# Patryk27/strolle

Hardware: NVIDIA H100
Metric: Mrays/s (+ frames/s) at 1080p-per-GPU Cornell, ReSTIR DI+GI + SVGF; H100 vs CPU restatement of the reference (higher is better)
Workload: dtype f32

## Files before the change

strolle_b200/csrc/engine.cu:

```cuda
#include <algorithm>
#include <cmath>
#include <cstdio>
#include <cstring>
#include <deque>
#include <functional>
#include <limits>
#include <string>
#include <unordered_map>
#include <vector>

#include <nccl.h>

#include "../../include/strolle_b200.h"
#include "kernels.h"

#include <dlfcn.h>
namespace {
struct NcclApi {
    void* lib = nullptr;
    ncclResult_t (*GetUniqueId)(ncclUniqueId*) = nullptr;
    ncclResult_t (*CommInitRank)(ncclComm_t*, int, ncclUniqueId, int) = nullptr;
    ncclResult_t (*CommDestroy)(ncclComm_t) = nullptr;
    ncclResult_t (*GroupStart)() = nullptr;
    ncclResult_t (*GroupEnd)() = nullptr;
// ... 305 lines not shown
    void* p = nullptr; size_t cap = 0;
    int ensure(size_t bytes) {
        if (bytes <= cap) return ST_OK;
        if (p) cudaFree(p);
        p = nullptr; cap = 0;
        size_t want = std::max<size_t>(bytes, 256);
        CK(cudaMalloc(&p, want));
        CK(cudaMemset(p, 0, want));
        CK(cudaDeviceSynchronize());
        cap = want;
        return ST_OK;
    }
    void release() { if (p) cudaFree(p); p = nullptr; cap = 0; }
};

static const char* kPassNames[P_COUNT] = {
    "prim_gbuffer", "di_sampling", "di_temporal_resampling", "di_spatial_resampling_pick", "di_spatial_resampling_trace", "di_spatial_resampling_sample",
    "di_resolving", "gi_reprojection", "gi_sampling_a", "gi_sampling_b", "gi_temporal_resampling", "gi_spatial_resampling_pick",
    "gi_spatial_resampling_trace", "gi_spatial_resampling_sample", "gi_preview_resampling", "gi_resolving", "frame_reprojection",
    "frame_denoising_reproject", "frame_denoising_estimate_variance", "frame_denoising_wavelet", "frame_composition", "ref_tracing",
    "ref_shading", "bvh_heatmap", "atmosphere", "trace_stream", "halo_exchange"};

static uint32_t dispatch_seed(uint32_t base, uint32_t frame, uint32_t k) {
    uint32_t s = base ^ (frame * 64u + k);
    s = s * 747796405u + 2891336453u;
    uint32_t w = ((s >> ((s >> 28) + 4u)) ^ s) * 277803737u;
    return (w >> 22) ^ w;
}

static const ExposureDev kExposureDefaults = {0.0f, 0.0f, -8.0f, 8.0f, 0.1f, 0.9f, 0.05f, 1.0f / 60.0f};
static const BloomDev kBloomDefaults = {0.15f, 0.7f, 0.0f, 0.0f, 7, 0};
static const st_depth_of_field kDofDefaults = {10.0f, 1.0f, 0.01866f, 16.0f};

struct CameraSlot {
    bool alive = false;
    st_camera desc;
    st_camera prev_desc;
    uint32_t frame = 0;
    CameraDev dev;
    std::vector<std::pair<std::string, float4**>> named;
    std::vector<std::pair<std::string, size_t>> sizes;
    DevMem arena;
    DevMem svgf_pairs; float4* pair[2] = {nullptr, nullptr};
    DevMem rgba8; int rgba8_slot = 0;
    DevMem taa; float4* taa_hist[2] = {nullptr, nullptr};
    DevMem expo;
    DevMem bloom;
    DevMem dof;
    cudaEvent_t ev_ready[2] = {nullptr, nullptr}, ev_copied[2] = {nullptr, nullptr};
    cudaStream_t side[2] = {nullptr, nullptr}; cudaEvent_t ev_produced = nullptr, ev_pushed[2] = {nullptr, nullptr}; bool pushed_pending[2] = {false, false};
    struct PeerLink { bool ready = false; bool ipc = false; std::vector<char*> arena, rgba8; std::vector<uint32_t*> flags; DevMem sync; uint32_t seq = 0, fseq = 0; } peer;
};

struct Step { int pass; std::function<void(cudaStream_t)> run; int sub = -1; };

}

using namespace st;

struct st_engine {
    int device = 0;
    cudaStream_t stream = nullptr; bool own_stream = true;
    cudaStream_t copy_stream = nullptr;
    std::unordered_map<st_handle, std::vector<st_mesh_triangle>> meshes;
    std::vector<st_material> materials; std::vector<st_handle> material_handles; bool materials_dirty = false;
    struct MatTex { st_handle tex[4]; uint32_t mask; };
    std::vector<MatTex> material_textures;
    struct ImageRect { st_handle handle; uint32_t x, y, w, h; };
    std::vector<ImageRect> images; uint32_t shelf_x = 0, shelf_y = 0, shelf_h = 0; bool images_dirty = false;
    DevMem d_atlas, d_srgb, d_tri_instance, d_instance_xforms;
    bool motion_dirty = true;
    bool moved_last_tick = false;
    struct Inst {
        st_handle handle, mesh, material; Affine3 xf, xf_inv, prev_xf; bool dirty;
        st_handle baked_mesh = ~(st_handle)0, baked_material = ~(st_handle)0; bool host_stale = false; Affine3 dev_xf, dev_xf_inv;
    };
    std::vector<Inst> instances; bool instances_dirty = false;
    struct Range { st_handle handle; size_t b, e; };
    std::vector<Range> tri_ranges; SlotAllocator tri_alloc;
    std::vector<float4> h_triangles; std::vector<Prim> prims; bool triangles_dirty = false;
    BvhBuild bvh; BvhOut bvh_out; bool bvh_dirty = false;
    std::vector<GpuMaterial> h_materials;
    static const st_handle kSun = ~(st_handle)0;
    std::vector<GpuLight> h_lights; std::vector<std::pair<st_handle, uint32_t>> light_slots;
    std::vector<st_handle> lights_created, lights_updated; std::vector<std::pair<st_handle, uint32_t>> lights_remapped; std::vector<uint32_t> lights_killed;
    uint32_t next_light = 1; bool lights_dirty = true;
    float sun_azimuth = 0.0f, sun_altitude = 0.35f; bool sun_dirty = true;
    GpuWorld world;
    uint32_t frame = 1, seed_base = 0xC0FFEEu;
    DevMem d_triangles, d_bvh, d_materials, d_matpacked, d_unpacklut, d_lights, d_noise, d_tlut, d_slut, d_skylut, d_scratch, d_raycount;
    bool count_rays = false;
    bool svgf_fast = true;
    bool shading_fast = ST_SHADING_FAST_DEFAULT != 0;
    bool fused_passes = ST_FUSED_PASSES_DEFAULT != 0;
    bool async_output = false;
    bool halo_nccl = false;
    int wavelet_paired = ST_WAVELET_PAIRED_DEFAULT;
    int strip_dma = ST_STRIP_DMA_DEFAULT;
    bool strip_fused = true;
    bool last_frame_fused = false;
    int wavelet_tiled = ST_WAVELET_TILED_DEFAULT;
    int wavelet_cfg = ST_WAVELET_CFG_DEFAULT;
    DevMem d_tile_errors; uint64_t wavelet_tiled_launches = 0;
    bool fuse_reproject = ST_FUSE_REPROJECT_DEFAULT != 0;
    bool bvh_reuse = true;
    bool variance_tiled = ST_VARIANCE_TILED_DEFAULT != 0; uint64_t variance_tiled_launches = 0;
    bool normal_maps = false, any_normal_map = false, nmap_frame = false; uint64_t normal_map_launches = 0;
    int bvh_refit = 0; uint32_t refit_run = 0; uint64_t bvh_refits = 0; bool structure_changed = false;
    RefitPlan plan; bool plan_ready = false; std::vector<uint32_t> plan_levels; std::vector<uint8_t> plan_alpha; DevMem d_plan, d_bake;
    std::unordered_map<st_handle, DevMem> d_meshes;
    void* staging[2] = {nullptr, nullptr}; size_t staging_cap[2] = {0, 0}; cudaEvent_t staging_ev[2] = {nullptr, nullptr}; int staging_slot = 0;
    int light_grid = 0, lgrid_built = 0; bool lgrid_frame = false; LightGridDev lgrid{}; DevMem d_lgrid; uint64_t light_grid_builds = 0;
    bool texture_filter = false, texf_built = false, any_color_texture = false, texf_frame = false; TexFilterDev texf{};
    DevMem d_texf_pool, d_texf_table, d_texf_jobs; std::vector<uint2> h_texf_table; std::vector<MipJob> h_texf_jobs; size_t texf_pool_texels = 0;
    uint64_t texture_mip_builds = 0;
    bool temporal_aa = false, taa_frame = false; uint64_t taa_resolves = 0;
// ... 521 lines not shown
    const double fx = -(double)c.transform[8], fy = -(double)c.transform[9], fz = -(double)c.transform[10];
    const double n = std::sqrt(fx * fx + fy * fy + fz * fz);
    DofDev p = {};
    p.active = active ? 1 : 0; p.k = (float)k; p.F = l.focal_distance; p.R = l.max_radius;
    p.fwd_x = (float)(fx / n); p.fwd_y = (float)(fy / n); p.fwd_z = (float)(fz / n);
    p.reach = (int)std::ceil((double)l.max_radius / kDofTile);
    const DofBufs b = dof_bufs(cs);
    const float fl[8] = {(float)f, (float)A, p.k, p.F, p.R, p.fwd_x, p.fwd_y, p.fwd_z};
    p.head[0] = c.width; p.head[1] = c.height; p.head[2] = (uint32_t)b.tx; p.head[3] = (uint32_t)b.ty; p.head[4] = (uint32_t)p.active;
    std::memcpy(p.head + 5, fl, sizeof fl);
    return p;
}
static bool lens_params(const st_engine* e, const CameraSlot* cs, uint32_t seed, LensDev* out) {
    const st_depth_of_field& l = e->dof_cfg;
    const st_camera& c = cs->desc;
    const double f = 0.5 * (double)l.sensor_height * (double)c.projection[5], A = f / (double)l.aperture_f_stops;
    if (!(e->dof_frame && c.mode == ST_MODE_REFERENCE && (double)l.focal_distance > f)) return false;
    double ax[3][3];
    for (int k = 0; k < 3; k++) {
        const double sg = k == 2 ? -1.0 : 1.0;
        const double x = sg * c.transform[4 * k], y = sg * c.transform[4 * k + 1], z = sg * c.transform[4 * k + 2], n = std::sqrt(x * x + y * y + z * z);
        ax[k][0] = x / n; ax[k][1] = y / n; ax[k][2] = z / n;
    }
    *out = LensDev{seed, (float)(A / 2.0), l.focal_distance, (float)ax[0][0], (float)ax[0][1], (float)ax[0][2], (float)ax[1][0], (float)ax[1][1],
                   (float)ax[1][2], (float)ax[2][0], (float)ax[2][1], (float)ax[2][2]};
    return true;
}
static CameraDev frame_source(const st_engine* e, const CameraSlot* cs, CameraDev c) {
    if (defocuses(e, cs) && cs->dof.p) c.output = dof_bufs(cs).frame;
    return c;
}
static void build_schedule(st_engine* e, CameraSlot* cs, std::vector<Step>* steps, const StripExt* ext = nullptr) {
    GpuCamera jc, jp; float4 jit;
    const bool taa = taa_cameras(e, cs, &jc, &jp, &jit);
    const CameraDev cam = [&] { CameraDev c = cs->dev; if (taa) { c.curr = jc; c.prev = jp; } return c; }();
    const StripExt no_ext; const StripExt& x = ext ? *ext : no_ext;
    const CameraDev camG = grown(cam, x.gbuffer), camV = grown(cam, x.variance);
    const int pm0 = x.preview_mirror[0], pm1 = x.preview_mirror[1];
    const SceneDev sc = e->scene();
    const uint32_t f = cs->frame;
    const int cur = (f % 2u) == 1u ? 1 : 0;
    const st_camera& d = cs->desc;
    const bool fs = e->shading_fast;
    const bool nm = e->nmap_frame;
    const bool lgon = e->lgrid_frame;
    const LightGridDev lgd = e->lgrid;
    const bool tfon = e->texf_frame;
    const TexFilterDev tfd = e->texf;
    const bool emon = e->envm_frame;
    EnvMapDev emd = e->envm;
    if (!e->envs_frame) emd.cdf = nullptr;
    const bool eson = emon && e->envs_frame;
    auto seed = [&](uint32_t k) { return dispatch_seed(e->seed_base, f, k); };
    auto add = [&](int pass, std::function<void(cudaStream_t)> fn) { steps->push_back(Step{pass, std::move(fn)}); };
    const CameraDev camO = frame_source(e, cs, cam);
    auto defocus = [&]() {
        if (!defocuses(e, cs)) return;
        const DofDev dp = dof_params(e, cs); const DofBufs db = dof_bufs(cs);
        add(P_COMPOSITION, [=](cudaStream_t s) { e->dof_gathers++; launch_depth_of_field(cam, dp, db, s); });
    };
    auto meter = [&]() {
        if (!meters(e, cs)) return;
        uint32_t* state = (uint32_t*)cs->expo.p; const ExposureDev ep = e->expo_frame; const int sms = e->sm_count;
        add(P_COMPOSITION, [=](cudaStream_t s) { e->exposure_meterings++; launch_exposure_histogram(camO, state, ep, sms, s); });
    };
    auto pyramid = [&]() {
        if (!blooms(e, cs)) return;
        const BloomLevels lv = bloom_levels(e, cs); const uint32_t* state = meters(e, cs) ? (const uint32_t*)cs->expo.p : nullptr;
        const ExposureDev ep = e->expo_frame; const int tm = e->tm_frame; const BloomDev bp = e->bloom_cfg;
        add(P_COMPOSITION, [=](cudaStream_t s) { e->bloom_pyramids++; launch_bloom_pyramid(camO, lv, state, ep, tm, bp, s); });
    };
    const float4* di_final = (d.denoise && (d.mode == ST_MODE_IMAGE || d.mode == ST_MODE_DI_DIFFUSE)) ? cam.di_diff_curr_colors : cam.di_diff_samples;
    const float4* gi_final = (d.denoise && (d.mode == ST_MODE_IMAGE || d.mode == ST_MODE_GI_DIFFUSE)) ? cam.gi_diff_curr_colors : cam.gi_diff_samples;
    if (d.mode == ST_MODE_BVH_HEATMAP) {
        add(P_BVH_HEATMAP, [=](cudaStream_t s) { launch_bvh_heatmap(cam, sc, s); });
        add(P_COMPOSITION, [=](cudaStream_t s) { launch_composition(cam, sc, cur, 5u, di_final, gi_final, s); });
        return;
    }
    if (d.mode == ST_MODE_REFERENCE) {
        LensDev lens;
        const bool lon = lens_params(e, cs, seed(K_LENS), &lens);
        for (uint32_t depth = 0; depth <= (uint32_t)d.ref_depth; depth++) {
            uint32_t sd = seed(P_REF_SHADING_SEED + depth);
            add(P_REF_TRACING, [=](cudaStream_t s) { if (nm) e->normal_map_launches++; launch_ref_tracing(cam, sc, depth, nm, lon ? &lens : nullptr, s); });
            add(P_REF_SHADING, [=](cudaStream_t s) {
                if (emon) e->envm_launches++;
                launch_ref_shading(cam, sc, sd, depth, lgon ? &lgd : nullptr, tfon ? &tfd : nullptr, emon ? &emd : nullptr, lon ? &lens : nullptr, s);
            });
        }
        add(P_REF_SHADING, [=](cudaStream_t s) { launch_ref_shading(cam, sc, 0u, 255u, nullptr, nullptr, nullptr, nullptr, s); });
        add(P_COMPOSITION, [=](cudaStream_t s) { launch_composition(cam, sc, cur, 6u, di_final, gi_final, s); });
        meter(); pyramid();
        return;
    }
    const bool needs_di = d.mode == ST_MODE_IMAGE || d.mode == ST_MODE_DI_DIFFUSE || d.mode == ST_MODE_DI_SPECULAR;
    const bool needs_gi = d.mode == ST_MODE_IMAGE || d.mode == ST_MODE_GI_DIFFUSE || d.mode == ST_MODE_GI_SPECULAR;
    const int k4_in_k0 = (e->fused_passes && (ext == nullptr || ext->still) && !e->instances.empty()) ? 1 : 0;
    add(P_PRIM_GBUFFER, [=](cudaStream_t s) { if (nm) e->normal_map_launches++; launch_prim_gbuffer(camG, sc, cur, k4_in_k0, nm, tfon ? &tfd : nullptr, s); });
    const bool fp = e->fused_passes;
    if (!e->instances.empty()) {
        if (!k4_in_k0) add(P_FRAME_REPROJECTION, [=](cudaStream_t s) { launch_frame_reprojection(cam, sc, cur, s); });
        if (needs_di) {
            uint32_t s1 = seed(P_DI_SAMPLING), s2 = seed(P_DI_TEMPORAL), s3 = seed(P_DI_SPATIAL_PICK), s5 = seed(P_DI_SPATIAL_SAMPLE);
            if (fp) {
                add(P_DI_TEMPORAL, [=](cudaStream_t s) { (fs ? stf::launch_di_sample_temporal : st::launch_di_sample_temporal)(cam, sc, cur, s1, s2, f, lgon ? &lgd : nullptr, s); });
                add(P_DI_SPATIAL_PICK, [=](cudaStream_t s) { (fs ? stf::launch_di_spatial_fused : st::launch_di_spatial_fused)(cam, sc, cur, s3, s5, f, s); });
            } else {
                add(P_DI_SAMPLING, [=](cudaStream_t s) { (fs ? stf::launch_di_sampling : st::launch_di_sampling)(cam, sc, cur, s1, f, lgon ? &lgd : nullptr, s); });
                add(P_DI_TEMPORAL, [=](cudaStream_t s) { (fs ? stf::launch_di_temporal : st::launch_di_temporal)(cam, sc, cur, s2, s); });
                add(P_DI_SPATIAL_PICK, [=](cudaStream_t s) { (fs ? stf::launch_di_spatial_pick : st::launch_di_spatial_pick)(cam, sc, cur, s3, f, s); });
                add(P_DI_SPATIAL_TRACE, [=](cudaStream_t s) { (fs ? stf::launch_spatial_trace : st::launch_spatial_trace)(cam, sc, cam.di_diff_samples, cam.di_diff_curr_colors, cam.di_diff_stash, s); });
                add(P_DI_SPATIAL_SAMPLE, [=](cudaStream_t s) { (fs ? stf::launch_di_spatial_sample : st::launch_di_spatial_sample)(cam, sc, s5, f, s); });
            }
            add(P_DI_RESOLVING, [=](cudaStream_t s) { if (emon) e->envm_launches++; (fs ? stf::launch_di_resolving : st::launch_di_resolving)(cam, sc, cur, emon ? &emd : nullptr, s); });
        }
        if (needs_gi) {
            uint32_t sa = seed(P_GI_SAMPLING_A), sb = seed(P_GI_SAMPLING_B), st_ = seed(P_GI_TEMPORAL), sp = seed(P_GI_SPATIAL_PICK), ss = seed(P_GI_SPATIAL_SAMPLE), sv = seed(P_GI_PREVIEW);
            uint32_t source;
            const bool tracing = f % 6u < 4u;
            const int inline_rp = (fp && tracing) ? 1 : 0;
            if (!inline_rp) add(P_GI_REPROJECTION, [=](cudaStream_t s) { (fs ? stf::launch_gi_reprojection : st::launch_gi_reprojection)(cam, sc, cur, s); });
            auto sampling = [&]() {
                if (fp) {
                    add(P_GI_SAMPLING_B, [=](cudaStream_t s) {
                        if (nm) e->normal_map_launches++;
                        if (emon) e->envm_launches++;
                        (fs ? stf::launch_gi_sampling_fused : st::launch_gi_sampling_fused)(cam, sc, cur, sa, sb, f, nm, lgon ? &lgd : nullptr, tfon ? &tfd : nullptr, emon ? &emd : nullptr, s);
                    });
                    return;
                }
                add(P_GI_SAMPLING_A, [=](cudaStream_t s) {
                    if (nm) e->normal_map_launches++;
                    if (eson) e->envm_launches++;
                    (fs ? stf::launch_gi_sampling_a : st::launch_gi_sampling_a)(cam, sc, cur, sa, f, nm, tfon ? &tfd : nullptr, eson ? &emd : nullptr, s);
                });
                add(P_GI_SAMPLING_B, [=](cudaStream_t s) { if (emon) e->envm_launches++; (fs ? stf::launch_gi_sampling_b : st::launch_gi_sampling_b)(cam, sc, cur, sb, f, lgon ? &lgd : nullptr, emon ? &emd : nullptr, s); });
            };
            if (tracing) {
                if (f % 2u == 0u) sampling();
                add(P_GI_TEMPORAL, [=](cudaStream_t s) { (fs ? stf::launch_gi_temporal : st::launch_gi_temporal)(cam, sc, cur, st_, f, inline_rp, s); });
                if (f % 2u == 1u) {
                    if (fp) add(P_GI_SPATIAL_PICK, [=](cudaStream_t s) { (fs ? stf::launch_gi_spatial_fused : st::launch_gi_spatial_fused)(cam, sc, cur, sp, ss, f, s); });
                    else {
                        add(P_GI_SPATIAL_PICK, [=](cudaStream_t s) { (fs ? stf::launch_gi_spatial_pick : st::launch_gi_spatial_pick)(cam, sc, cur, sp, f, s); });
                        add(P_GI_SPATIAL_TRACE, [=](cudaStream_t s) { (fs ? stf::launch_spatial_trace : st::launch_spatial_trace)(cam, sc, cam.gi_d0, cam.gi_d1, cam.gi_d2, s); });
                        add(P_GI_SPATIAL_SAMPLE, [=](cudaStream_t s) { (fs ? stf::launch_gi_spatial_sample : st::launch_gi_spatial_sample)(cam, sc, ss, f, s); });
                    }
                    source = 1;
                } else source = 0;
            } else {
                sampling();
                add(P_GI_TEMPORAL, [=](cudaStream_t s) { (fs ? stf::launch_gi_temporal : st::launch_gi_temporal)(cam, sc, cur, st_, f, 0, s); });
                source = 0;
            }
            const float4* src0 = source == 0 ? cam.gi_reservoirs[1] : cam.gi_reservoirs[2];
            add(P_GI_PREVIEW, [=](cudaStream_t s) { (fs ? stf::launch_gi_preview : st::launch_gi_preview)(cam, sc, cur, sv, 0u, src0, cam.gi_reservoirs[3], pm0, s); });
            if (fp) add(P_GI_PREVIEW, [=](cudaStream_t s) { (fs ? stf::launch_gi_preview_resolve : st::launch_gi_preview_resolve)(cam, sc, cur, sv, cam.gi_reservoirs[3], src0, s); });
            else {
                add(P_GI_PREVIEW, [=](cudaStream_t s) { (fs ? stf::launch_gi_preview : st::launch_gi_preview)(cam, sc, cur, sv, 1u, cam.gi_reservoirs[3], cam.gi_reservoirs[0], pm1, s); });
                add(P_GI_RESOLVING, [=](cudaStream_t s) { (fs ? stf::launch_gi_resolving : st::launch_gi_resolving)(cam, sc, cur, src0, s); });
            }
        }
    }
    if (d.denoise) {
        if (e->fuse_reproject) {
            add(P_DENOISE_REPROJECT, [=](cudaStream_t s) { launch_denoise_reproject_pair(cam, sc, cur, s); });
        } else {
            add(P_DENOISE_REPROJECT, [=](cudaStream_t s) { launch_denoise_reproject(cam, sc, cur, cam.di_diff_prev_colors, cam.di_diff_moments[cur ^ 1], cam.di_diff_samples, cam.di_diff_curr_colors, cam.di_diff_moments[cur], s); });
            add(P_DENOISE_REPROJECT, [=](cudaStream_t s) { launch_denoise_reproject(cam, sc, cur, cam.gi_diff_prev_colors, cam.gi_diff_moments[cur ^ 1], cam.gi_diff_samples, cam.gi_diff_curr_colors, cam.gi_diff_moments[cur], s); });
        }
        const bool fast = e->svgf_fast;
        const bool var_tiled = e->variance_tiled; uint32_t* verr = (uint32_t*)e->d_tile_errors.p;
        add(P_DENOISE_VARIANCE, [=](cudaStream_t s) {
            if (var_tiled && launch_denoise_variance_tiled(camV, sc, cur, fast, verr, s)) { e->variance_tiled_launches++; return; }
            launch_denoise_variance(camV, sc, cur, fast, s);
        });
        float4* di_io[5][2] = {{cam.di_diff_stash, cam.di_diff_prev_colors}, {cam.di_diff_prev_colors, cam.di_diff_stash}, {cam.di_diff_stash, cam.di_diff_curr_colors},
                               {cam.di_diff_curr_colors, cam.di_diff_stash}, {cam.di_diff_stash, cam.di_diff_curr_colors}};
        float4* gi_io[5][2] = {{cam.gi_diff_stash, cam.gi_diff_prev_colors}, {cam.gi_diff_prev_colors, cam.gi_diff_stash}, {cam.gi_diff_stash, cam.gi_diff_curr_colors},
                               {cam.gi_diff_curr_colors, cam.gi_diff_stash}, {cam.gi_diff_stash, cam.gi_diff_curr_colors}};
        const bool whole_or_fused = ext != nullptr || (cam.y0 == 0 && cam.y1 == cam.h);
        const int first_paired_read = (fast && whole_or_fused && cs->pair[0]) ? (e->wavelet_paired == 2 ? 3 : e->wavelet_paired == 1 ? 4 : 5) : 5;
        for (uint32_t nth = 0; nth < 5; nth++) {
            float4 *a = di_io[nth][0], *b = di_io[nth][1], *c = gi_io[nth][0], *g = gi_io[nth][1];
            const bool reads_pair = (int)nth >= first_paired_read, writes_pair = (int)nth + 1 >= first_paired_read && nth < 4;
            const float4* pin = reads_pair ? cs->pair[nth & 1] : nullptr; float4* pout = writes_pair ? cs->pair[(nth + 1) & 1] : nullptr;
            const bool tiled = !reads_pair && ((e->wavelet_tiled >> nth) & 1) != 0; const int cfg = (e->wavelet_cfg >> (4 * nth)) & 15;
            uint32_t* terr = (uint32_t*)e->d_tile_errors.p;
            const CameraDev camW = grown(cam, x.wavelet[nth]);
            add(P_DENOISE_WAVELET, [=](cudaStream_t s) {
                if (tiled && launch_denoise_wavelet_tiled(camW, sc, f, 1u << nth, (float)(1 + nth), a, b, c, g, pout, fast, cfg, terr, s)) { e->wavelet_tiled_launches++; return; }
                launch_denoise_wavelet(camW, sc, cur, f, 1u << nth, (float)(1 + nth), a, b, c, g, pin, pout, fast, s);
            });
            steps->back().sub = (int)nth;
        }
    }
    uint32_t mode = (uint32_t)d.mode;
    if (taa) {
        const float4* hin = cs->taa_hist[cur ^ 1]; float4* hout = cs->taa_hist[cur];
        add(P_COMPOSITION, [=](cudaStream_t s) { e->taa_resolves++; launch_taa_resolve(cam, sc, cur, mode, di_final, gi_final, hin, hout, jit, s); });
        defocus(); meter(); pyramid();
        return;
    }
    add(P_COMPOSITION, [=](cudaStream_t s) { launch_composition(cam, sc, cur, mode, di_final, gi_final, s); });
    defocus(); meter(); pyramid();
}


struct HaloItem { std::string name; int reach; };
struct HaloExchange { int before_step; std::vector<HaloItem> items; };
static const int kSpatialReach = 128;
static const int kPreview2Reach = 64;
static const int kVarianceReach = 3;
static const int kWaveletReach[5] = {1, 2, 4, 9, 19};

// ... 259 lines not shown
            break;
        case StripOp::PULL: {
            StripPull pl; std::memset(&pl, 0, sizeof pl);
            for (int r = 0; r < N; r++) { pl.arena[r] = cs->peer.arena[r]; pl.bounds[r] = bounds[r].first; }
            pl.bounds[N] = H; pl.n_ranks = N; pl.rank = R; pl.w = (int)cs->desc.width; pl.h = H; pl.own_y0 = d.own_y0; pl.own_y1 = d.own_y1;
            pl.need_rows = (const int*)(sync + kNeedRowsWord); pl.pulled_rows = (unsigned long long*)(sync + kPulledRowsWord);
            struct { std::string name; int local; } items[] = {
                {std::string("prim_surface_map_") + prv, kSpatialReach}, {std::string("prim_gbuffer_d0_") + prv, kSpatialReach}, {std::string("prim_gbuffer_d1_") + prv, kSpatialReach},
                {"di_reservoirs_0", 0}, {"gi_reservoirs_0", 0}, {"di_diff_prev_colors", 0}, {"gi_diff_prev_colors", 0},
                {std::string("di_diff_moments_") + prv, 0}, {std::string("gi_diff_moments_") + prv, 0}};
            for (auto& it : items) {
                size_t kk = 0; float4* base = camera_buffer(cs, it.name, &kk);
                if (!base) return fail(ST_ERR_NOT_FOUND, "pull list names unknown buffer " + it.name);
                pl.items[pl.nitems++] = StripPullItem{(size_t)((char*)base - (char*)cs->arena.p), (int)kk, it.local};
            }
            e->run_timed(P_HALO_EXCHANGE, [=](cudaStream_t s) { launch_strip_pull(pl, s); });
            break;
        }
        }
    }
    d.y0 = d.own_y0; d.y1 = d.own_y1;
    if (push_rc) return push_rc;
    CK(cudaGetLastError());
    return ST_OK;
}

static CameraSlot* get_camera(st_engine* e, st_camera_handle h) { return (h >= 0 && (size_t)h < e->cameras.size() && e->cameras[h]->alive) ? e->cameras[h] : nullptr; }

}

extern "C" {

int st_copy_output(st_engine* e, st_camera_handle h, void* host_out, int format);
const char* st_last_error(void) { return g_err.c_str(); }
const char* st_pass_name(int pass) { return (pass >= 0 && pass < P_COUNT) ? kPassNames[pass] : ""; }

int st_engine_create(int device, st_engine** out) {
    if (!out) return fail(ST_ERR_INVALID, "out is null");
    int count = 0;
    cudaError_t ce = cudaGetDeviceCount(&count);
    if (ce != cudaSuccess || count == 0) return fail(ST_ERR_CUDA, "no CUDA device available: this library has no CPU fallback");
    if (device < 0 || device >= count) return fail(ST_ERR_INVALID, "bad device ordinal");
    CK(cudaSetDevice(device));
    st_engine* e = new st_engine();
    e->device = device;
    CK(cudaDeviceGetAttribute(&e->sm_count, cudaDevAttrMultiProcessorCount, device));
    CK(cudaStreamCreateWithFlags(&e->stream, cudaStreamNonBlocking));
    std::memset(&e->world, 0, sizeof e->world);
    e->h_lights.push_back(make_sun(make_float4(0, 0, 0, 25.0f), make_float4(0, 0, 0, std::numeric_limits<float>::infinity())));
    e->light_slots.push_back({st_engine::kSun, 0u});
    int rc = e->d_noise.ensure(256 * 256 * 4); if (rc) { delete e; return rc; }
    rc = e->d_unpacklut.ensure(512 * 4); if (rc) { delete e; return rc; }
    rc = e->d_tile_errors.ensure(4); if (rc) { delete e; return rc; }
    launch_unpack_lut((float*)e->d_unpacklut.p, e->stream);
    *out = e;
    return ST_OK;
}
void st_engine_destroy(st_engine* e) {
    if (!e) return;
    cudaSetDevice(e->device);
    cudaStreamSynchronize(e->stream);
    if (e->copy_stream) cudaStreamSynchronize(e->copy_stream);
    for (CameraSlot* c : e->cameras) { for (int k = 0; k < 2; k++) { if (c->side[k]) { cudaStreamSynchronize(c->side[k]); cudaStreamDestroy(c->side[k]); } if (c->ev_pushed[k]) cudaEventDestroy(c->ev_pushed[k]); } if (c->ev_produced) cudaEventDestroy(c->ev_produced);
        c->arena.release(); c->svgf_pairs.release(); c->rgba8.release(); for (int k = 0; k < 2; k++) { if (c->ev_ready[k]) cudaEventDestroy(c->ev_ready[k]); if (c->ev_copied[k]) cudaEventDestroy(c->ev_copied[k]); } delete c; }
    DevMem* all[] = {&e->d_triangles, &e->d_bvh, &e->d_materials, &e->d_lights, &e->d_noise, &e->d_tlut, &e->d_slut, &e->d_skylut, &e->d_scratch, &e->d_raycount, &e->d_matpacked, &e->d_unpacklut, &e->d_atlas, &e->d_srgb, &e->d_tri_instance, &e->d_instance_xforms, &e->d_tile_errors, &e->d_plan, &e->d_bake, &e->d_lgrid, &e->d_texf_pool, &e->d_texf_table, &e->d_texf_jobs, &e->d_envm, &e->d_envs};
    for (DevMem* d : all) d->release();
    for (auto& m : e->d_meshes) m.second.release();
    for (int k = 0; k < 2; k++) { if (e->staging[k]) cudaFreeHost(e->staging[k]); if (e->staging_ev[k]) cudaEventDestroy(e->staging_ev[k]); }
    for (auto& t : e->pending) { cudaEventDestroy(t.a); cudaEventDestroy(t.b); }
    for (cudaEvent_t ev : e->event_pool) cudaEventDestroy(ev);
    if (e->comm) g_nccl.CommDestroy(e->comm);
    if (e->own_stream) cudaStreamDestroy(e->stream);
    if (e->copy_stream) cudaStreamDestroy(e->copy_stream);
    delete e;
}

int st_insert_mesh(st_engine* e, st_handle mesh, const st_mesh_triangle* tris, size_t count) {
    if (!e || (!tris && count)) return fail(ST_ERR_INVALID, "null argument");
    rebake_host_mesh(e, mesh);
    auto dm = e->d_meshes.find(mesh);
    if (dm != e->d_meshes.end()) { cudaSetDevice(e->device); dm->second.release(); e->d_meshes.erase(dm); }
    e->meshes[mesh].assign(tris, tris + count);
    return ST_OK;
}
int st_remove_mesh(st_engine* e, st_handle mesh) {
    if (!e) return fail(ST_ERR_INVALID, "null engine");
    rebake_host_mesh(e, mesh);
    auto dm = e->d_meshes.find(mesh);
    if (dm != e->d_meshes.end()) { cudaSetDevice(e->device); dm->second.release(); e->d_meshes.erase(dm); }
    e->meshes.erase(mesh);
    return ST_OK;
}

int st_insert_material(st_engine* e, st_handle h, const st_material* m) {
    if (!e || !m) return fail(ST_ERR_INVALID, "null argument");
    auto it = std::find(e->material_handles.begin(), e->material_handles.end(), h);
    if (it != e->material_handles.end()) e->materials[it - e->material_handles.begin()] = *m;
    else { e->material_handles.push_back(h); e->materials.push_back(*m); st_engine::MatTex mt; std::memset(&mt, 0, sizeof mt); e->material_textures.push_back(mt); }
    e->materials_dirty = true;
    return ST_OK;
}
int st_has_material(st_engine* e, st_handle h) { return e && std::find(e->material_handles.begin(), e->material_handles.end(), h) != e->material_handles.end() ? 1 : 0; }
int st_remove_material(st_engine* e, st_handle h) {
    if (!e) return fail(ST_ERR_INVALID, "null engine");
    auto it = std::find(e->material_handles.begin(), e->material_handles.end(), h);
    if (it != e->material_handles.end()) *it = ~(st_handle)0 - 1;
    e->materials_dirty = true;
    return ST_OK;
}

int st_insert_image(st_engine* e, st_handle h, const uint8_t* rgba8, uint32_t w, uint32_t hgt) {
    if (!e || !rgba8 || w == 0 || hgt == 0) return fail(ST_ERR_INVALID, "null argument");
    CK(cudaSetDevice(e->device));
    int rc;
    if (!e->d_atlas.p) {
        if ((rc = e->d_atlas.ensure((size_t)kAtlasSize * kAtlasSize * 4))) return rc;
        if ((rc = e->d_srgb.ensure(256 * 4))) return rc;
        launch_srgb_lut((float*)e->d_srgb.p, e->stream);
    }
    st_engine::ImageRect* r = nullptr;
    for (auto& k : e->images) if (k.handle == h) r = &k;
    if (!r || r->w != w || r->h != hgt) {
        if (e->shelf_x + w > kAtlasSize) { e->shelf_x = 0; e->shelf_y += e->shelf_h; e->shelf_h = 0; }
        if (w > kAtlasSize || e->shelf_y + hgt > kAtlasSize) return fail(ST_ERR_LIMIT, "no more space in the atlas");
        st_engine::ImageRect nr = {h, e->shelf_x, e->shelf_y, w, hgt};
        e->shelf_x += w; if (hgt > e->shelf_h) e->shelf_h = hgt;
// ... 244 lines not shown
    else if (lights_uploaded || e->lgrid_built != e->light_grid) { if ((rc = build_light_grid(e))) return rc; }
    e->lgrid_frame = e->light_grid > 0;
    for (CameraSlot* c : e->cameras) if (c->alive) c->frame = e->frame;
    e->nmap_frame = e->normal_maps && e->any_normal_map;
    if (!e->texture_filter) {
        if (e->texf_built || e->d_texf_pool.p) { e->d_texf_pool.release(); e->d_texf_table.release(); e->d_texf_jobs.release(); e->texf = TexFilterDev{}; }
        e->texf_built = false;
    } else if (textures_changed || !e->texf_built) { if ((rc = build_texture_mips(e))) return rc; }
    e->texf_frame = e->texture_filter && e->any_color_texture;
    if (e->envm_dirty) {
        e->envm_dirty = false;
        if (e->envm_set) {
            const size_t bytes = e->h_envm.size() * sizeof(float4);
            if ((rc = upload(e, e->d_envm, e->h_envm.data(), bytes))) return rc;
            e->envm.texels = (const float4*)e->d_envm.p; e->envm.w = e->envm_w; e->envm.h = e->envm_h;
            e->envm.intensity = e->envm_intensity; e->envm.rotation = e->envm_rotation;
        } else { e->d_envm.release(); e->envm = EnvMapDev{}; }
        if (e->envm_new_texels || !e->envm_set) e->envs_built = false;
        e->envm_new_texels = false;
    }
    e->envm_frame = e->envm_set;
    if (!(e->envm_sampling && e->envm_set)) { e->d_envs.release(); e->envs_built = false; e->envm.cdf = nullptr; e->envm.total = 0.0f; }
    else if (!e->envs_built) { if ((rc = build_env_distribution(e))) return rc; }
    e->envs_frame = e->envs_built && e->envm.total > 0.0f && e->envm.total < INFINITY;
    if (e->temporal_aa != e->taa_frame) for (CameraSlot* c : e->cameras) { c->taa.release(); c->taa_hist[0] = c->taa_hist[1] = nullptr; }
    e->taa_frame = e->temporal_aa;
    if ((e->tonemapping != 0 && e->auto_exposure) != (e->tm_frame != 0 && e->ae_frame)) for (CameraSlot* c : e->cameras) c->expo.release();
    e->tm_frame = e->tonemapping; e->ae_frame = e->auto_exposure; e->expo_frame = e->exposure;
    if (e->bloom != e->bloom_frame || e->bloom_set.levels != e->bloom_cfg.levels) for (CameraSlot* c : e->cameras) c->bloom.release();
    e->bloom_frame = e->bloom; e->bloom_cfg = e->bloom_set;
    if (e->dof != e->dof_frame) for (CameraSlot* c : e->cameras) c->dof.release();
    e->dof_frame = e->dof; e->dof_cfg = e->dof_set;
    e->frame += 1;
    if (too_deep) return fail(ST_ERR_LIMIT, "BVH deeper than the 24-entry traversal stack (strolle-gpu/src/lib.rs:72-76): the scene is not drawn until it changes");
    return ST_OK;
}

int st_frame_schedule(st_engine* e, st_camera_handle h, int* pass_ids, int cap, int* count) {
    CameraSlot* cs = e ? get_camera(e, h) : nullptr;
    if (!cs || !count) return fail(ST_ERR_NOT_FOUND, "unknown camera");
    std::vector<Step> steps; build_schedule(e, cs, &steps);
    *count = (int)steps.size();
    for (int i = 0; i < cap && i < *count; i++) pass_ids[i] = steps[i].pass;
    return ST_OK;
}
static int ensure_taa_history(st_engine* e, CameraSlot* cs) {
    GpuCamera a, b; float4 j;
    if (cs->taa.p || !taa_cameras(e, cs, &a, &b, &j)) return ST_OK;
    const size_t bytes = ((size_t)cs->desc.width * cs->desc.height * 16 + 255) / 256 * 256;
    int rc = cs->taa.ensure(2 * bytes); if (rc) return rc;
    cs->taa_hist[0] = (float4*)cs->taa.p; cs->taa_hist[1] = (float4*)((char*)cs->taa.p + bytes);
    return ST_OK;
}
int st_render_range(st_engine* e, st_camera_handle h, int first, int last) {
    CameraSlot* cs = e ? get_camera(e, h) : nullptr;
    if (!cs) return fail(ST_ERR_NOT_FOUND, "unknown camera");
    if (cs->frame == 0) return fail(ST_ERR_INVALID, "st_tick must precede st_render_camera");
    CK(cudaSetDevice(e->device));
    int rc = ensure_luts(e); if (rc) return rc;
    if ((rc = ensure_taa_history(e, cs))) return rc;
    if ((rc = ensure_exposure_state(e, cs))) return rc;
    if ((rc = ensure_bloom_state(e, cs))) return rc;
    if ((rc = ensure_dof_state(e, cs))) return rc;
    std::vector<Step> steps; build_schedule(e, cs, &steps);
    if (last < 0 || last >= (int)steps.size()) last = (int)steps.size() - 1;
    for (int i = std::max(first, 0); i <= last; i++) e->run_timed(steps[i].pass, steps[i].run, steps[i].sub);
    CK(cudaGetLastError());
    return ST_OK;
}
int st_render_camera(st_engine* e, st_camera_handle h, void* host_out, int format) {
    int rc = st_render_range(e, h, 0, -1); if (rc) return rc;
    if (host_out) return st_copy_output(e, h, host_out, format);
    return ST_OK;
}
static int store_rgba8(st_engine* e, CameraSlot* cs, const CameraDev& cd, uchar4* dst8) {
    const SceneDev sc = e->scene();
    const int op = cs->desc.mode == ST_MODE_BVH_HEATMAP ? 0 : e->tm_frame;
    if (blooms(e, cs)) {
        int rc = ensure_exposure_state(e, cs); if (rc) return rc;
        if ((rc = ensure_bloom_state(e, cs))) return rc;
        const uint32_t* state = meters(e, cs) ? (const uint32_t*)cs->expo.p : nullptr; const ExposureDev ep = e->expo_frame;
        const BloomDev bp = e->bloom_cfg; const BloomLevels lv = bloom_levels(e, cs);
        e->run_timed(P_COMPOSITION, [=](cudaStream_t s) { launch_output_bloom(cd, sc, op, state, ep, bp, lv.up[0], lv.w[0], lv.h[0], dst8, s); });
        return ST_OK;
    }
    if (op == 0) { e->run_timed(P_COMPOSITION, [=](cudaStream_t s) { launch_output_rgba8(cd, sc, dst8, s); }); return ST_OK; }
    int rc = ensure_exposure_state(e, cs); if (rc) return rc;
    const uint32_t* state = meters(e, cs) ? (const uint32_t*)cs->expo.p : nullptr; const ExposureDev ep = e->expo_frame;
    e->run_timed(P_COMPOSITION, [=](cudaStream_t s) { launch_output_display(cd, sc, op, state, ep, dst8, s); });
    return ST_OK;
}
static int copy_rows_out(st_engine* e, CameraSlot* cs, void* host_out, int format, int y0, int y1) {
    const size_t W = cs->desc.width, n = W * cs->desc.height;
    const size_t first = (size_t)y0 * W, count = (size_t)(y1 - y0) * W;
    int rc2 = ensure_dof_state(e, cs); if (rc2) return rc2;
    const CameraDev src = frame_source(e, cs, cs->dev);
    if (format == ST_FORMAT_RGBA32F) CK(cudaMemcpyAsync((char*)host_out + first * 16, src.output + first, count * 16, cudaMemcpyDeviceToHost, e->stream));
    else if (format == ST_FORMAT_RGBA8_SRGB) {
        if ((rc2 = cs->rgba8.ensure(2 * n * 4))) return rc2;
        cs->rgba8_slot ^= 1;
        uchar4* dst8 = (uchar4*)cs->rgba8.p + (cs->rgba8_slot ? n : 0); CameraDev cd = src; cd.y0 = y0; cd.y1 = y1;
        const int k = cs->rgba8_slot;
        if (e->async_output) {
            if (!e->copy_stream) CK(cudaStreamCreateWithFlags(&e->copy_stream, cudaStreamNonBlocking));
            if (!cs->ev_ready[k]) { CK(cudaEventCreateWithFlags(&cs->ev_ready[k], cudaEventDisableTiming)); CK(cudaEventCreateWithFlags(&cs->ev_copied[k], cudaEventDisableTiming)); }
            else CK(cudaStreamWaitEvent(e->stream, cs->ev_copied[k], 0));
        }
        if ((rc2 = store_rgba8(e, cs, cd, dst8))) return rc2;
        if (e->async_output) {
            CK(cudaEventRecord(cs->ev_ready[k], e->stream));
            CK(cudaStreamWaitEvent(e->copy_stream, cs->ev_ready[k], 0));
            CK(cudaMemcpyAsync((char*)host_out + first * 4, dst8 + first, count * 4, cudaMemcpyDeviceToHost, e->copy_stream));
            CK(cudaEventRecord(cs->ev_copied[k], e->copy_stream));
        } else CK(cudaMemcpyAsync((char*)host_out + first * 4, dst8 + first, count * 4, cudaMemcpyDeviceToHost, e->stream));
    } else return fail(ST_ERR_INVALID, "unsupported output format");
    return ST_OK;
}
int st_copy_output(st_engine* e, st_camera_handle h, void* host_out, int format) {
    CameraSlot* cs = e ? get_camera(e, h) : nullptr;
// ... 628 lines not shown
static int link_prepare(st_engine* e, CameraSlot* cs) {
    CK(cudaSetDevice(e->device));
    size_t n = (size_t)cs->desc.width * cs->desc.height;
    int rc = cs->rgba8.ensure(2 * n * 4); if (rc) return rc;
    if ((rc = cs->peer.sync.ensure(kSyncBytes))) return rc;
    const int need0[2] = {(int)cs->desc.height, -1};
    CK(cudaMemcpy((uint32_t*)cs->peer.sync.p + kNeedRowsWord, need0, 8, cudaMemcpyHostToDevice));
    return ST_OK;
}
int st_link_local(st_engine* const* engines, const st_camera_handle* cameras, int n) {
    if (!engines || !cameras || n < 1 || n > ST_PEER_MAX_RANKS) return fail(ST_ERR_LIMIT, "1..16 engines");
    std::vector<CameraSlot*> cams(n);
    for (int r = 0; r < n; r++) {
        cams[r] = engines[r] ? get_camera(engines[r], cameras[r]) : nullptr;
        if (!cams[r]) return fail(ST_ERR_NOT_FOUND, "unknown camera");
        if (cams[r]->desc.width != cams[0]->desc.width || cams[r]->desc.height != cams[0]->desc.height) return fail(ST_ERR_INVALID, "linked cameras must have one size");
        int rc = link_prepare(engines[r], cams[r]); if (rc) return rc;
    }
    for (int a = 0; a < n; a++) for (int b = 0; b < n; b++) {
        if (engines[a]->device == engines[b]->device) continue;
        int can = 0; CK(cudaDeviceCanAccessPeer(&can, engines[a]->device, engines[b]->device));
        if (!can) return fail(ST_ERR_CUDA, "devices cannot access each other's memory");
        CK(cudaSetDevice(engines[a]->device));
        cudaError_t ce = cudaDeviceEnablePeerAccess(engines[b]->device, 0);
        if (ce != cudaSuccess && ce != cudaErrorPeerAccessAlreadyEnabled) return fail(ST_ERR_CUDA, std::string("cudaDeviceEnablePeerAccess: ") + cudaGetErrorString(ce));
        cudaGetLastError();
    }
    for (int r = 0; r < n; r++) {
        CameraSlot* cs = cams[r];
        cs->peer.arena.assign(n, nullptr); cs->peer.rgba8.assign(n, nullptr); cs->peer.flags.assign(n, nullptr);
        for (int q = 0; q < n; q++) { cs->peer.arena[q] = (char*)cams[q]->arena.p; cs->peer.flags[q] = (uint32_t*)cams[q]->peer.sync.p; cs->peer.rgba8[q] = (char*)cams[q]->rgba8.p; }
        engines[r]->rank = r; engines[r]->n_ranks = n; cs->peer.seq = 0; cs->peer.fseq = 0; cs->peer.ready = true; cs->peer.ipc = false;
    }
    for (int r = 0; r < n; r++) { int rc = strip_streams_prepare(engines[r], cams[r]); if (rc) return rc; }
    return ST_OK;
}
int st_halo_bytes(st_engine* e, uint64_t* bytes) { if (!e || !bytes) return fail(ST_ERR_INVALID, "null argument"); *bytes = e->halo_bytes_last_frame; return ST_OK; }
int st_mark_begin(st_engine* e) {
    if (!e) return fail(ST_ERR_INVALID, "null engine");
    CK(cudaSetDevice(e->device));
    if (!e->mark_a) { CK(cudaEventCreate(&e->mark_a)); CK(cudaEventCreate(&e->mark_b)); }
    CK(cudaEventRecord(e->mark_a, e->stream));
    return ST_OK;
}
int st_mark_end(st_engine* e, float* ms) {
    if (!e || !ms || !e->mark_a) return fail(ST_ERR_INVALID, "st_mark_begin first");
    CK(cudaSetDevice(e->device));
    CK(cudaEventRecord(e->mark_b, e->stream));
    CK(cudaEventSynchronize(e->mark_b));
    CK(cudaEventElapsedTime(ms, e->mark_a, e->mark_b));
    return ST_OK;
}
int st_enable_timing(st_engine* e, int enabled) { if (!e) return fail(ST_ERR_INVALID, "null engine"); e->timing = enabled != 0; return ST_OK; }
int st_pass_times(st_engine* e, float* ms, uint32_t* launches, int reset) {
    if (!e) return fail(ST_ERR_INVALID, "null engine");
    CK(cudaSetDevice(e->device));
    e->collect_timing();
    for (int i = 0; i < P_COUNT; i++) { if (ms) ms[i] = e->pass_ms[i]; if (launches) launches[i] = e->pass_launches[i]; }
    if (reset) { std::memset(e->pass_ms, 0, sizeof e->pass_ms); std::memset(e->pass_launches, 0, sizeof e->pass_launches); }
    return ST_OK;
}

int st_wavelet_times(st_engine* e, float* ms5, uint32_t* launches5, int reset) {
    if (!e) return fail(ST_ERR_INVALID, "null engine");
    CK(cudaSetDevice(e->device));
    e->collect_timing();
    for (int i = 0; i < 5; i++) { if (ms5) ms5[i] = e->wavelet_ms[i]; if (launches5) launches5[i] = e->wavelet_launches[i]; }
    if (reset) { std::memset(e->wavelet_ms, 0, sizeof e->wavelet_ms); std::memset(e->wavelet_launches, 0, sizeof e->wavelet_launches); }
    return ST_OK;
}

struct st_multi { std::vector<st_engine*> e; std::vector<std::vector<st_camera_handle>> cams; };
#define ST_MULTI_ALL(call) do { if (!m) return fail(ST_ERR_INVALID, "null group"); for (st_engine* e : m->e) { int rc_ = (call); if (rc_) return rc_; } return ST_OK; } while (0)
int st_multi_create(const int* devices, int n, st_multi** out) {
    if (!devices || !out || n < 1 || n > ST_PEER_MAX_RANKS) return fail(ST_ERR_LIMIT, "1..16 devices");
    st_multi* m = new st_multi();
    for (int i = 0; i < n; i++) { st_engine* e = nullptr; int rc = st_engine_create(devices[i], &e); if (rc) { for (st_engine* x : m->e) st_engine_destroy(x); delete m; return rc; } m->e.push_back(e); }
    *out = m;
    return ST_OK;
}
void st_multi_destroy(st_multi* m) { if (!m) return; for (st_engine* e : m->e) { cudaSetDevice(e->device); cudaStreamSynchronize(e->stream); } for (st_engine* e : m->e) st_engine_destroy(e); delete m; }
int st_multi_size(st_multi* m) { return m ? (int)m->e.size() : 0; }
st_engine* st_multi_engine(st_multi* m, int rank) { return (m && rank >= 0 && rank < (int)m->e.size()) ? m->e[rank] : nullptr; }
int st_multi_insert_mesh(st_multi* m, st_handle mesh, const st_mesh_triangle* t, size_t count) { ST_MULTI_ALL(st_insert_mesh(e, mesh, t, count)); }
int st_multi_remove_mesh(st_multi* m, st_handle mesh) { ST_MULTI_ALL(st_remove_mesh(e, mesh)); }
int st_multi_insert_material(st_multi* m, st_handle h, const st_material* mat) { ST_MULTI_ALL(st_insert_material(e, h, mat)); }
int st_multi_has_material(st_multi* m, st_handle h) { return (m && !m->e.empty()) ? st_has_material(m->e[0], h) : 0; }
int st_multi_remove_material(st_multi* m, st_handle h) { ST_MULTI_ALL(st_remove_material(e, h)); }
int st_multi_insert_image(st_multi* m, st_handle h, const uint8_t* rgba8, uint32_t w, uint32_t hgt) { ST_MULTI_ALL(st_insert_image(e, h, rgba8, w, hgt)); }
int st_multi_remove_image(st_multi* m, st_handle h) { ST_MULTI_ALL(st_remove_image(e, h)); }
int st_multi_set_material_textures(st_multi* m, st_handle h, const st_material_textures* t) { ST_MULTI_ALL(st_set_material_textures(e, h, t)); }
int st_multi_insert_instance(st_multi* m, st_handle h, st_handle mesh, st_handle material, const float a[12]) { ST_MULTI_ALL(st_insert_instance(e, h, mesh, material, a)); }
int st_multi_remove_instance(st_multi* m, st_handle h) { ST_MULTI_ALL(st_remove_instance(e, h)); }
int st_multi_insert_light(st_multi* m, st_handle h, const st_light* l) { ST_MULTI_ALL(st_insert_light(e, h, l)); }
int st_multi_remove_light(st_multi* m, st_handle h) { ST_MULTI_ALL(st_remove_light(e, h)); }
int st_multi_update_sun(st_multi* m, float az, float alt) { ST_MULTI_ALL(st_update_sun(e, az, alt)); }
int st_multi_set_environment_map(st_multi* m, const float* rgba32f, uint32_t width, uint32_t height, float intensity, float rotation) {
    ST_MULTI_ALL(st_set_environment_map(e, rgba32f, width, height, intensity, rotation));
}
int st_multi_set_option(st_multi* m, int option, int value) { ST_MULTI_ALL(st_set_option(e, option, value)); }
int st_multi_set_exposure(st_multi* m, const st_exposure* x) {
    ExposureDev v; int rc = exposure_from(x, &v); if (rc) return rc;
    ST_MULTI_ALL(st_set_exposure(e, x));
}
int st_multi_set_bloom(st_multi* m, const st_bloom* x) {
    BloomDev v; int rc = bloom_from(x, &v); if (rc) return rc;
// ... 88 lines not shown
```

Before: 3732.

## Run ReSTIR DI chain on a side stream concurrently with GI chain

Tags schedule steps as DI, GI or frame chains and, for single-rank full-frame image renders with timing off, launches the DI passes on a separate non-blocking stream forked from the main stream. The GI passes stay on the main stream, and the two streams join before the next frame-level pass such as denoising. The aim is to overlap the independent DI and GI work so the GPU is busier when individual kernels underfill it. This relies on DI and GI passes not sharing buffers they write. It adds event fork/join overhead and a debug toggle to force serial execution.

```diff
diff --git a/strolle_b200/csrc/engine.cu b/strolle_b200/csrc/engine.cu
--- a/strolle_b200/csrc/engine.cu
+++ b/strolle_b200/csrc/engine.cu
@@ -381,7 +381,8 @@
     struct PeerLink { bool ready = false; bool ipc = false; std::vector<char*> arena, rgba8; std::vector<uint32_t*> flags; DevMem sync; uint32_t seq = 0, fseq = 0; } peer;
 };
 
-struct Step { int pass; std::function<void(cudaStream_t)> run; int sub = -1; };
+enum Chain { CHAIN_FRAME = 0, CHAIN_DI = 1, CHAIN_GI = 2 };
+struct Step { int pass; std::function<void(cudaStream_t)> run; int sub = -1; int chain = CHAIN_FRAME; };
 
 }
 
@@ -391,6 +392,7 @@
     int device = 0;
     cudaStream_t stream = nullptr; bool own_stream = true;
     cudaStream_t copy_stream = nullptr;
+    cudaStream_t di_stream = nullptr; cudaEvent_t di_fork = nullptr, di_join = nullptr; bool serial_chains = false; uint64_t overlapped_frames = 0;
     std::unordered_map<st_handle, std::vector<st_mesh_triangle>> meshes;
     std::vector<st_material> materials; std::vector<st_handle> material_handles; bool materials_dirty = false;
     struct MatTex { st_handle tex[4]; uint32_t mask; };
@@ -1018,7 +1020,8 @@
     if (!e->envs_frame) emd.cdf = nullptr;
     const bool eson = emon && e->envs_frame;
     auto seed = [&](uint32_t k) { return dispatch_seed(e->seed_base, f, k); };
-    auto add = [&](int pass, std::function<void(cudaStream_t)> fn) { steps->push_back(Step{pass, std::move(fn)}); };
+    int chain = CHAIN_FRAME;
+    auto add = [&](int pass, std::function<void(cudaStream_t)> fn) { steps->push_back(Step{pass, std::move(fn), -1, chain}); };
     const CameraDev camO = frame_source(e, cs, cam);
     auto defocus = [&]() {
         if (!defocuses(e, cs)) return;
@@ -1067,6 +1070,7 @@
     if (!e->instances.empty()) {
         if (!k4_in_k0) add(P_FRAME_REPROJECTION, [=](cudaStream_t s) { launch_frame_reprojection(cam, sc, cur, s); });
         if (needs_di) {
+            chain = CHAIN_DI;
             uint32_t s1 = seed(P_DI_SAMPLING), s2 = seed(P_DI_TEMPORAL), s3 = seed(P_DI_SPATIAL_PICK), s5 = seed(P_DI_SPATIAL_SAMPLE);
             if (fp) {
                 add(P_DI_TEMPORAL, [=](cudaStream_t s) { (fs ? stf::launch_di_sample_temporal : st::launch_di_sample_temporal)(cam, sc, cur, s1, s2, f, lgon ? &lgd : nullptr, s); });
@@ -1081,6 +1085,7 @@
             add(P_DI_RESOLVING, [=](cudaStream_t s) { if (emon) e->envm_launches++; (fs ? stf::launch_di_resolving : st::launch_di_resolving)(cam, sc, cur, emon ? &emd : nullptr, s); });
         }
         if (needs_gi) {
+            chain = CHAIN_GI;
             uint32_t sa = seed(P_GI_SAMPLING_A), sb = seed(P_GI_SAMPLING_B), st_ = seed(P_GI_TEMPORAL), sp = seed(P_GI_SPATIAL_PICK), ss = seed(P_GI_SPATIAL_SAMPLE), sv = seed(P_GI_PREVIEW);
             uint32_t source;
             const bool tracing = f % 6u < 4u;
@@ -1127,6 +1132,7 @@
                 add(P_GI_RESOLVING, [=](cudaStream_t s) { (fs ? stf::launch_gi_resolving : st::launch_gi_resolving)(cam, sc, cur, src0, s); });
             }
         }
+        chain = CHAIN_FRAME;
     }
     if (d.denoise) {
         if (e->fuse_reproject) {
@@ -1492,6 +1498,8 @@
     int rc = e->d_noise.ensure(256 * 256 * 4); if (rc) { delete e; return rc; }
     rc = e->d_unpacklut.ensure(512 * 4); if (rc) { delete e; return rc; }
     rc = e->d_tile_errors.ensure(4); if (rc) { delete e; return rc; }
+    CK(cudaStreamCreateWithFlags(&e->di_stream, cudaStreamNonBlocking));
+    CK(cudaEventCreateWithFlags(&e->di_fork, cudaEventDisableTiming)); CK(cudaEventCreateWithFlags(&e->di_join, cudaEventDisableTiming));
     launch_unpack_lut((float*)e->d_unpacklut.p, e->stream);
     *out = e;
     return ST_OK;
@@ -1512,6 +1520,9 @@
     if (e->comm) g_nccl.CommDestroy(e->comm);
     if (e->own_stream) cudaStreamDestroy(e->stream);
     if (e->copy_stream) cudaStreamDestroy(e->copy_stream);
+    if (e->di_stream) { cudaStreamSynchronize(e->di_stream); cudaStreamDestroy(e->di_stream); }
+    if (e->di_fork) cudaEventDestroy(e->di_fork);
+    if (e->di_join) cudaEventDestroy(e->di_join);
     delete e;
 }
 
@@ -1862,6 +1873,28 @@
     cs->taa_hist[0] = (float4*)cs->taa.p; cs->taa_hist[1] = (float4*)((char*)cs->taa.p + bytes);
     return ST_OK;
 }
+static bool overlaps_chains(const st_engine* e, const CameraSlot* cs) {
+    const CameraDev& d = cs->dev;
+    return !e->serial_chains && !e->timing && e->n_ranks == 1 && cs->desc.mode == ST_MODE_IMAGE && d.y0 == 0 && d.y1 == d.h && d.own_y0 == 0 &&
+           d.own_y1 == d.h && d.mirror_up == 0 && d.mirror_dn == 0 && d.need_rows == nullptr;
+}
+static int render_overlapped(st_engine* e, const std::vector<Step>& steps) {
+    bool forked = false, joined = false;
+    auto join = [&]() -> int { CK(cudaEventRecord(e->di_join, e->di_stream)); CK(cudaStreamWaitEvent(e->stream, e->di_join, 0)); joined = true; return ST_OK; };
+    int rc = ST_OK;
+    for (const Step& st : steps) {
+        if (st.chain == CHAIN_DI) {
+            if (!forked) { CK(cudaEventRecord(e->di_fork, e->stream)); CK(cudaStreamWaitEvent(e->di_stream, e->di_fork, 0)); forked = true; }
+            st.run(e->di_stream); e->pass_launches[st.pass]++;
+            continue;
+        }
+        if (forked && !joined && st.chain == CHAIN_FRAME && (rc = join())) return rc;
+        e->run_timed(st.pass, st.run, st.sub);
+    }
+    if (forked && !joined && (rc = join())) return rc;
+    if (forked) e->overlapped_frames++;
+    return ST_OK;
+}
 int st_render_range(st_engine* e, st_camera_handle h, int first, int last) {
     CameraSlot* cs = e ? get_camera(e, h) : nullptr;
     if (!cs) return fail(ST_ERR_NOT_FOUND, "unknown camera");
@@ -1874,7 +1907,8 @@
     if ((rc = ensure_dof_state(e, cs))) return rc;
     std::vector<Step> steps; build_schedule(e, cs, &steps);
     if (last < 0 || last >= (int)steps.size()) last = (int)steps.size() - 1;
-    for (int i = std::max(first, 0); i <= last; i++) e->run_timed(steps[i].pass, steps[i].run, steps[i].sub);
+    if (first <= 0 && last == (int)steps.size() - 1 && overlaps_chains(e, cs)) { if ((rc = render_overlapped(e, steps))) return rc; }
+    else for (int i = std::max(first, 0); i <= last; i++) e->run_timed(steps[i].pass, steps[i].run, steps[i].sub);
     CK(cudaGetLastError());
     return ST_OK;
 }
@@ -2609,6 +2643,12 @@
     return ST_OK;
 }
 int st_enable_timing(st_engine* e, int enabled) { if (!e) return fail(ST_ERR_INVALID, "null engine"); e->timing = enabled != 0; return ST_OK; }
+int st_debug_serial_chains(st_engine* e, int serial, uint64_t* overlapped_frames) {
+    if (!e) return fail(ST_ERR_INVALID, "null engine");
+    e->serial_chains = serial != 0;
+    if (overlapped_frames) *overlapped_frames = e->overlapped_frames;
+    return ST_OK;
+}
 int st_pass_times(st_engine* e, float* ms, uint32_t* launches, int reset) {
     if (!e) return fail(ST_ERR_INVALID, "null engine");
     CK(cudaSetDevice(e->device));
```

After: 3854, median of 6. 3.3% higher.
